# NoahVl/Explaining-In-Style-Reproducibility-Study

Measured on AMD Instinct MI355X. Metric: StylEx G+D+enc train-step images/sec @256px, higher is better.
Workload: dtype bf16; 1 GPU; FFHQ-shaped 256x256 StylEx, batch 32/GPU, GAE=2 (noise+encoder micro-steps), GP every 4th step, ResNet-18 classifier; image_size=256, batch_per_gpu=32, start_step=0, gradient_accumulate_every=2, global_batch=32, parallelism=dp1

## Files before the change

### explaining-in-style-reproducibility-study_amd/csrc/elementwise.hip

```cpp
#include <hip/hip_runtime.h>
#include <stdint.h>

#include "stylex_internal.h"

namespace {

template <int V>
struct Vec;
template <>
struct Vec<4> {
    typedef float4 T;
    static __device__ __forceinline__ T zero() { return make_float4(0.f, 0.f, 0.f, 0.f); }
    static __device__ __forceinline__ T ld(const void* p, long off, int bf) { return act_ld4(p, off, bf); }
    static __device__ __forceinline__ void st(void* p, long off, T v, int bf) { act_st4(p, off, v, bf); }
    static __device__ __forceinline__ void fma(T& a, float w, T x) {
        a.x = fmaf(w, x.x, a.x); a.y = fmaf(w, x.y, a.y); a.z = fmaf(w, x.z, a.z); a.w = fmaf(w, x.w, a.w);
    }
};
template <>
struct Vec<1> {
    typedef float T;
    static __device__ __forceinline__ T zero() { return 0.f; }
    static __device__ __forceinline__ T ld(const void* p, long off, int bf) { return act_ld1(p, off, bf); }
    static __device__ __forceinline__ void st(void* p, long off, T v, int bf) { act_st1(p, off, v, bf); }
// ... 99 lines not shown
            float ch = up_coef(oh, ih, H);
            if (ch == 0.f) continue;
#pragma unroll
            for (int e = -1; e <= 2; ++e) {
                int ow = 2 * iw + e;
                if (ow < 0 || ow >= 2 * W) continue;
                float cw = up_coef(ow, iw, W);
                if (cw == 0.f) continue;
                Vec<V>::fma(acc, ch * cw, Vec<V>::ld(dy, base + ((long)oh * 2 * W + ow) * C, bf));
            }
        }
        Vec<V>::st(dx, pix * C + c, acc, bf);
    }
}

__device__ __forceinline__ int reflect1(int i, int n) { return i < 0 ? -i : (i >= n ? 2 * n - 2 - i : i); }

__device__ __forceinline__ float ub_coef(int o, int i, int n) {
    const int n2 = 2 * n;
    return 0.25f * up_coef(reflect1(o - 1, n2), i, n) + 0.5f * up_coef(o, i, n) + 0.25f * up_coef(reflect1(o + 1, n2), i, n);
}

template <int V>
__global__ void rgb_up_blur_add_fwd_kernel(const void* __restrict__ rgb, const void* __restrict__ prev, void* __restrict__ y,
                                           int B, int H, int W, int C, int bf) {
    const int cv = C / V;
    const long total = (long)B * 2 * H * 2 * W * cv;
    for (long i = blockIdx.x * (long)blockDim.x + threadIdx.x; i < total; i += (long)gridDim.x * blockDim.x) {
        int cq, ow, oh, b;
        const long pix = decomp_index(i, cv, 2 * W, 2 * H, cq, ow, oh, b);
// ... 359 lines not shown
           ((reinterpret_cast<uintptr_t>(b) & 15) == 0);
}
template <bool ADJ>
static int launch_blur_strip(const void* in, void* out, int B, int H, int W, int C, int s2d, hipStream_t s,
                             const void* gate = nullptr, float gslope = 0.f, const void* gmask = nullptr) {
    constexpr int ROWS = 8;
    long work = (long)B * ((H + ROWS - 1) / ROWS) * W * (C / 8);
    long blocks = (work + 255) / 256;
    if (blocks > 16384) blocks = 16384;
    hipLaunchKernelGGL((blur3x3_strip_kernel<ADJ, ROWS>), dim3((unsigned)blocks), dim3(256), 0, s,
                       (const unsigned short*)in, (unsigned short*)out, B, H, W, C, s2d, (const unsigned short*)gate,
                       gslope, (const unsigned char*)gmask);
    return (int)hipGetLastError();
}

extern "C" {

#define EW_ARGS const int64_t* sh, int act_dtype, void* stream
#define EW_UNPACK                                                     \
    hipStream_t s = (hipStream_t)stream;                               \
    int B = (int)sh[0], H = (int)sh[1], W = (int)sh[2], C = (int)sh[3]; \
    int bf = act_dtype == 1;                                           \
    if (act_dtype != 0 && act_dtype != 1) return STYLEX_EINVAL;

int stylex_upsample2x_bilinear_fwd(const void* x, void* y, EW_ARGS) {
    EW_UNPACK
    if (B <= 0 || H <= 0 || W <= 0 || C <= 0) return STYLEX_EINVAL;
    LAUNCH_EW(upsample2x_fwd_kernel, (long)B * 4 * H * W * C, x, y, x, y, B, H, W, C, bf);
}
int stylex_upsample2x_bilinear_bwd(const void* dy, void* dx, EW_ARGS) {
    EW_UNPACK
    if (B <= 0 || H <= 0 || W <= 0 || C <= 0) return STYLEX_EINVAL;
    LAUNCH_EW(upsample2x_bwd_kernel, (long)B * H * W * C, dy, dx, dy, dx, B, H, W, C, bf);
}
int stylex_rgb_up_blur_add_fwd(const void* rgb, const void* prev, void* y, EW_ARGS) {
    EW_UNPACK
    if (!rgb || !y || B <= 0 || H <= 0 || W <= 0 || C <= 0) return STYLEX_EINVAL;
    const void* al = prev ? prev : rgb;
    if (vec_ok(C, rgb, y) && vec_ok(C, al, y))
        hipLaunchKernelGGL(rgb_up_blur_add_fwd_kernel<4>, dim3(grid_for((long)B * 4 * H * W * C / 4)), dim3(256), 0, s, rgb, prev,
                           y, B, H, W, C, bf);
    else
        hipLaunchKernelGGL(rgb_up_blur_add_fwd_kernel<1>, dim3(grid_for((long)B * 4 * H * W * C)), dim3(256), 0, s, rgb, prev, y,
                           B, H, W, C, bf);
    return (int)hipGetLastError();
}
int stylex_rgb_up_blur_add_bwd(const void* dy, void* dx, EW_ARGS) {
// ... 117 lines not shown
```

### explaining-in-style-reproducibility-study_amd/csrc/fused_bwd.hip

```cpp
#include <hip/hip_runtime.h>
#include <stdint.h>

#include "stylex_internal.h"

namespace {

constexpr int NT = 256;

template <int K>
struct Acc {
    float4 v[K];
    __device__ __forceinline__ void zero() {
#pragma unroll
        for (int k = 0; k < K; ++k) v[k] = make_float4(0.f, 0.f, 0.f, 0.f);
    }
};

template <int K>
__device__ __forceinline__ void block_reduce_store(Acc<K>& a, float* smem, int cv, int prow, int CV, int rpp, int C,
                                                   float* partial_row , bool active) {
    float4* s4 = reinterpret_cast<float4*>(smem);
    if (active) {
#pragma unroll
        for (int k = 0; k < K; ++k) s4[(k * rpp + prow) * CV + cv] = a.v[k];
// ... 30 lines not shown
    if (g.CV > NT) g.CV = NT;
    g.rpp = NT / g.CV;
    g.cv = threadIdx.x % g.CV;
    g.prow = threadIdx.x / g.CV;
    g.active = g.prow < g.rpp;
    g.b = blockIdx.y;
    long per = ((long)HW + nchunks - 1) / nchunks;
    g.p_begin = (long)blockIdx.x * per;
    g.p_end = g.p_begin + per < HW ? g.p_begin + per : HW;
    return g;
}

__device__ __forceinline__ float4 ld4(const void* p, long off, int bf) { return act_ld4(p, off, bf); }
__device__ __forceinline__ void st4(void* p, long off, float4 v, int bf) { act_st4(p, off, v, bf); }
__device__ __forceinline__ float4 ldp4(const float* p) { return *reinterpret_cast<const float4*>(p); }

__global__ __launch_bounds__(NT) void act_bwd_reduce_kernel(const void* __restrict__ dy, const void* __restrict__ y,
                                                           void* __restrict__ dx, float* __restrict__ partial, int HW,
                                                           int C, int nchunks, int lrelu, float scale, int bf) {
    extern __shared__ __attribute__((aligned(16))) float smem[];
    Geo g = make_geo(HW, C, nchunks);
    Acc<1> a;
    a.zero();
    const int c = g.cv * 4;
    if (g.active && c < C) {
        const long base = (long)g.b * HW;
        for (long p = g.p_begin + g.prow; p < g.p_end; p += g.rpp) {
            const long o = (base + p) * C + c;
            float4 gv = ld4(dy, o, bf);
            gv.x *= scale; gv.y *= scale; gv.z *= scale; gv.w *= scale;
// ... 6 lines not shown
                gv.w = yv.w > 0.f ? gv.w : slope * gv.w;
            }
            if (dx) st4(dx, o, gv, bf);
            a.v[0].x += gv.x; a.v[0].y += gv.y; a.v[0].z += gv.z; a.v[0].w += gv.w;
        }
    }
    block_reduce_store<1>(a, smem, g.cv, g.prow, g.CV, g.rpp, C, partial + ((long)g.b * nchunks + blockIdx.x) * C,
                          g.active && c < C);
}

__global__ __launch_bounds__(NT) void modconv_bwd_prep_kernel(const void* __restrict__ gy, const void* __restrict__ y,
                                                             const float* __restrict__ noise, int ns,
                                                             const float* __restrict__ nw, const float* __restrict__ nb,
                                                             void* __restrict__ gz, float* __restrict__ partial, int H,
                                                             int W, int C, int nchunks, int lrelu, int bf,
                                                             const float* __restrict__ gz_scale) {
    extern __shared__ __attribute__((aligned(16))) float smem[];
    const int HW = H * W;
    Geo g = make_geo(HW, C, nchunks);
    Acc<3> a;
    a.zero();
    const int c = g.cv * 4;
    if (g.active && c < C) {
        float4 w4 = make_float4(0.f, 0.f, 0.f, 0.f), b4 = w4;
        if (noise) {
            w4 = ldp4(nw + c);
            b4 = ldp4(nb + c);
        }
        float4 d4 = make_float4(1.f, 1.f, 1.f, 1.f);
        if (gz_scale) d4 = ldp4(gz_scale + (long)g.b * C + c);
        const long base = (long)g.b * HW;
        for (long p = g.p_begin + g.prow; p < g.p_end; p += g.rpp) {
            const long o = (base + p) * C + c;
            float4 gv = ld4(gy, o, bf);
            float4 yv = ld4(y, o, bf);
            float nz = 0.f;
            if (noise) {
                const int pi = (int)p, h = pi / W, w = pi - h * W;
                nz = noise[((long)g.b * ns + w) * ns + h];
            }
            float4 t = yv;
            if (lrelu) {
                gv.x = yv.x > 0.f ? gv.x : 0.2f * gv.x; t.x = yv.x > 0.f ? yv.x : 5.f * yv.x;
                gv.y = yv.y > 0.f ? gv.y : 0.2f * gv.y; t.y = yv.y > 0.f ? yv.y : 5.f * yv.y;
                gv.z = yv.z > 0.f ? gv.z : 0.2f * gv.z; t.z = yv.z > 0.f ? yv.z : 5.f * yv.z;
                gv.w = yv.w > 0.f ? gv.w : 0.2f * gv.w; t.w = yv.w > 0.f ? yv.w : 5.f * yv.w;
            }
            if (gz_scale) st4(gz, o, make_float4(gv.x * d4.x, gv.y * d4.y, gv.z * d4.z, gv.w * d4.w), bf);
            else st4(gz, o, gv, bf);
            a.v[0].x += gv.x * (t.x - (nz * w4.x + b4.x));
            a.v[0].y += gv.y * (t.y - (nz * w4.y + b4.y));
            a.v[0].z += gv.z * (t.z - (nz * w4.z + b4.z));
            a.v[0].w += gv.w * (t.w - (nz * w4.w + b4.w));
            a.v[1].x += gv.x * nz; a.v[1].y += gv.y * nz; a.v[1].z += gv.z * nz; a.v[1].w += gv.w * nz;
            a.v[2].x += gv.x; a.v[2].y += gv.y; a.v[2].z += gv.z; a.v[2].w += gv.w;
// ... 17 lines not shown
        for (long p = g.p_begin + g.prow; p < g.p_end; p += g.rpp) {
            const long o = (base + p) * C + c;
            float4 tv = ld4(t, o, bf);
            float4 xv = ld4(x, o, bf);
            a.v[0].x += xv.x * tv.x; a.v[0].y += xv.y * tv.y; a.v[0].z += xv.z * tv.z; a.v[0].w += xv.w * tv.w;
            if (gx) {
                tv.x *= s4.x; tv.y *= s4.y; tv.z *= s4.z; tv.w *= s4.w;
                st4(gx, o, tv, bf);
            }
        }
    }
    block_reduce_store<1>(a, smem, g.cv, g.prow, g.CV, g.rpp, C, partial + ((long)g.b * nchunks + blockIdx.x) * C,
                          g.active && c < C);
}

inline size_t reduce_smem(int C, int K) {
    int CV = (C + 3) / 4;
    if (CV > NT) CV = NT;
    int rpp = NT / CV;
    return (size_t)K * rpp * CV * 16;
}

inline bool ok_shape(const int64_t* sh, int nchunks) {
    return sh[0] > 0 && sh[1] > 0 && sh[2] > 0 && sh[3] > 0 && sh[3] <= 1024 && (sh[3] % 4 == 0) && nchunks > 0 &&
           sh[0] <= 65535;
}

}

extern "C" {
// ... 7 lines not shown
    return (int)n;
}

int stylex_act_bwd_reduce(const void* dy, const void* y, void* dx, float* partial, const int64_t* sh, int nchunks,
                          int lrelu, float scale, int act_dtype, void* stream) {
    if (act_dtype != 0 && act_dtype != 1) return STYLEX_EINVAL;
    if (!dy || !partial || !ok_shape(sh, nchunks) || (lrelu && !y)) return STYLEX_EINVAL;
    int HW = (int)(sh[1] * sh[2]), C = (int)sh[3];
    hipLaunchKernelGGL(act_bwd_reduce_kernel, dim3(nchunks, (unsigned)sh[0]), dim3(NT), reduce_smem(C, 1),
                       (hipStream_t)stream, dy, y, dx, partial, HW, C, nchunks, lrelu, scale, act_dtype);
    return (int)hipGetLastError();
}

static int modconv_bwd_prep_impl(const void* gy, const void* y, const float* noise, int64_t noise_stride,
                                 const float* noise_w, const float* noise_b, void* gz, float* partial, const int64_t* sh,
                                 int nchunks, int lrelu, int act_dtype, const float* gz_scale, void* stream);

int stylex_modconv_bwd_prep(const void* gy, const void* y, const float* noise, int64_t noise_stride,
                            const float* noise_w, const float* noise_b, void* gz, float* partial, const int64_t* sh,
                            int nchunks, int lrelu, int act_dtype, void* stream) {
    return modconv_bwd_prep_impl(gy, y, noise, noise_stride, noise_w, noise_b, gz, partial, sh, nchunks, lrelu, act_dtype,
                                 nullptr, stream);
}

int stylex_modconv_bwd_prep_scaled(const void* gy, const void* y, const float* noise, int64_t noise_stride,
                                   const float* noise_w, const float* noise_b, const float* gz_scale, void* gz,
                                   float* partial, const int64_t* sh, int nchunks, int lrelu, int act_dtype, void* stream) {
    if (!gz_scale || (reinterpret_cast<uintptr_t>(gz_scale) & 15)) return STYLEX_EINVAL;
    return modconv_bwd_prep_impl(gy, y, noise, noise_stride, noise_w, noise_b, gz, partial, sh, nchunks, lrelu, act_dtype,
                                 gz_scale, stream);
}

static int modconv_bwd_prep_impl(const void* gy, const void* y, const float* noise, int64_t noise_stride,
                                 const float* noise_w, const float* noise_b, void* gz, float* partial, const int64_t* sh,
                                 int nchunks, int lrelu, int act_dtype, const float* gz_scale, void* stream) {
    if (act_dtype != 0 && act_dtype != 1) return STYLEX_EINVAL;
    if (lrelu != 0 && lrelu != 1) return STYLEX_EINVAL;
    if (!gy || !y || !gz || !partial || !ok_shape(sh, nchunks)) return STYLEX_EINVAL;
    if (noise && (!noise_w || !noise_b || noise_stride < sh[1] || noise_stride < sh[2])) return STYLEX_EINVAL;
    int C = (int)sh[3];
    hipLaunchKernelGGL(modconv_bwd_prep_kernel, dim3(nchunks, (unsigned)sh[0]), dim3(NT), reduce_smem(C, 3),
                       (hipStream_t)stream, gy, y, noise, (int)noise_stride, noise_w, noise_b, gz, partial, (int)sh[1],
                       (int)sh[2], C, nchunks, lrelu, act_dtype, gz_scale);
    return (int)hipGetLastError();
}

int stylex_scale_reduce(const void* x, const void* t, const float* s, void* gx, float* partial, const int64_t* sh,
                        int nchunks, int act_dtype, void* stream) {
    if (act_dtype != 0 && act_dtype != 1) return STYLEX_EINVAL;
    if (!x || !t || !s || !partial || !ok_shape(sh, nchunks)) return STYLEX_EINVAL;
    int HW = (int)(sh[1] * sh[2]), C = (int)sh[3];
    hipLaunchKernelGGL(scale_reduce_kernel, dim3(nchunks, (unsigned)sh[0]), dim3(NT), reduce_smem(C, 1),
                       (hipStream_t)stream, x, t, s, gx, partial, HW, C, nchunks, act_dtype);
    return (int)hipGetLastError();
}

}
```

### explaining-in-style-reproducibility-study_amd/stylex/hip_backend.py

```python
import os as _os

if _os.environ.get("STYLEX_MIOPEN_ALLOW_BWD_GTC", "0") != "1":
    _os.environ.setdefault("MIOPEN_DEBUG_CONV_IMPLICIT_GEMM_ASM_BWD_GTC_XDLOPS_NHWC", "0")

import atexit
import ctypes
import os
import weakref

import torch

import operand_cache
from operand_cache import mark_updated, packs, stamp as _gen, vectors

_HERE = os.path.dirname(os.path.abspath(__file__))
LIB_PATH = os.path.join(os.path.dirname(_HERE), "libstylex_hip.so")

F32, BF16, BF16_ACT = 0, 1, 2
EPI_BIAS, EPI_LRELU, EPI_OSCALE, EPI_NOISE, EPI_RESIDUAL, EPI_RELU, EPI_GATE, EPI_NOISE_NAT = 1, 2, 4, 8, 16, 32, 64, 128
EPI_MASK_OUT, EPI_GATE_MASK = 256, 512

_c_f = ctypes.c_void_p
_i64p = ctypes.POINTER(ctypes.c_int64)

# ... 51 lines not shown
    "stylex_rgb_up_blur_add_fwd": (ctypes.c_int, [_c_f, _c_f, _c_f, _i64p, ctypes.c_int, ctypes.c_void_p]),
    "stylex_rgb_up_blur_add_bwd": (ctypes.c_int, [_c_f, _c_f, _i64p, ctypes.c_int, ctypes.c_void_p]),
    "stylex_blur3x3_reflect_fwd": (ctypes.c_int, [_c_f, _c_f, _i64p, ctypes.c_int, ctypes.c_void_p]),
    "stylex_blur3x3_reflect_bwd": (ctypes.c_int, [_c_f, _c_f, _i64p, ctypes.c_int, ctypes.c_void_p]),
    "stylex_bias_act_fwd": (ctypes.c_int, [_c_f, _c_f, _c_f, ctypes.c_int64, _c_f, _c_f, _c_f, _i64p, ctypes.c_int,
                                           ctypes.c_void_p]),
    "stylex_bias_act_bwd": (ctypes.c_int, [_c_f, _c_f, _c_f, _i64p, ctypes.c_int, ctypes.c_void_p]),
    "stylex_rowwise_sumsq": (ctypes.c_int, [_c_f, _c_f, _i64p, ctypes.c_void_p]),
    "stylex_reduce_chunks": (ctypes.c_int, [_i64p]),
    "stylex_act_bwd_reduce": (ctypes.c_int, [_c_f, _c_f, _c_f, _c_f, _i64p, ctypes.c_int, ctypes.c_int, ctypes.c_float,
                                             ctypes.c_int, ctypes.c_void_p]),
    "stylex_modconv_bwd_prep": (ctypes.c_int, [_c_f, _c_f, _c_f, ctypes.c_int64, _c_f, _c_f, _c_f, _c_f, _i64p,
                                               ctypes.c_int, ctypes.c_int, ctypes.c_int, ctypes.c_void_p]),
    "stylex_modconv_bwd_prep_scaled": (ctypes.c_int, [_c_f, _c_f, _c_f, ctypes.c_int64, _c_f, _c_f, _c_f, _c_f, _c_f, _i64p,
                                                      ctypes.c_int, ctypes.c_int, ctypes.c_int, ctypes.c_void_p]),
    "stylex_scale_reduce": (ctypes.c_int, [_c_f, _c_f, _c_f, _c_f, _c_f, _i64p, ctypes.c_int, ctypes.c_int,
                                           ctypes.c_void_p]),
    "stylex_pad_rgb8": (ctypes.c_int, [_c_f, _c_f, _i64p, _i64p, ctypes.c_int, ctypes.c_void_p]),
    "stylex_affine_act_nchw_fwd": (ctypes.c_int, [_c_f, _c_f, _c_f, _c_f, _c_f, ctypes.c_int64, ctypes.c_int64, ctypes.c_int64,
                                                  ctypes.c_int, ctypes.c_void_p]),
    "stylex_affine_act_nchw_bwd": (ctypes.c_int, [_c_f, _c_f, _c_f, _c_f, _c_f, ctypes.c_int64, ctypes.c_int64, ctypes.c_int64,
                                                  ctypes.c_int, ctypes.c_void_p]),
    "stylex_affine_relu_maxpool_fwd": (ctypes.c_int, [_c_f, _c_f, _c_f, _c_f, _c_f, ctypes.c_int64, ctypes.c_int64,
                                                      ctypes.c_int64, ctypes.c_int64, ctypes.c_void_p]),
    "stylex_affine_relu_maxpool_bwd": (ctypes.c_int, [_c_f, _c_f, _c_f, _c_f, ctypes.c_int64, ctypes.c_int64, ctypes.c_int64,
                                                      ctypes.c_int64, ctypes.c_void_p]),
    "stylex_lpips_tap_nhwc_fwd": (ctypes.c_int, [_c_f, _c_f, _c_f, _c_f, _c_f, _c_f, ctypes.c_int64, ctypes.c_int64, ctypes.c_int64,
                                                 ctypes.c_int64, ctypes.c_void_p]),
    "stylex_lpips_tap_nhwc_bwd": (ctypes.c_int, [_c_f, _c_f, _c_f, _c_f, _c_f, _c_f, _c_f, _c_f, ctypes.c_int64, ctypes.c_int64,
                                                 ctypes.c_int64, ctypes.c_void_p]),
# ... 64 lines not shown
                                               ctypes.c_void_p]),
    "stylex_crop_lut_u8": (ctypes.c_int, [ctypes.c_void_p, _c_f, ctypes.c_int64, ctypes.c_int64, ctypes.c_int64, _c_f,
                                          ctypes.c_int64, _c_f, _c_f, ctypes.c_int64, ctypes.c_void_p]),
    "stylex_timing_report": (ctypes.c_int, [ctypes.c_int, _i64p, ctypes.POINTER(ctypes.c_double),
                                            ctypes.POINTER(ctypes.c_double), ctypes.POINTER(ctypes.c_double)]),
}

_lib = None
_inited_devices = set()


class StylexHipError(RuntimeError):
    pass


def load_library(path=None):
    global _lib
    if _lib is not None:
        return _lib
    path = path or os.environ.get("STYLEX_HIP_LIB", LIB_PATH)
    if not os.path.isfile(path):
        raise StylexHipError("libstylex_hip.so not found at %s — run `python __graft_entry__.py build` "
                             "(there is no CPU fallback for the product path)" % path)
    lib = ctypes.CDLL(path)
    for name, (res, args) in SIGNATURES.items():
        fn = getattr(lib, name)
        fn.restype = res
        fn.argtypes = args
    if os.environ.get("STYLEX_SYNC_TRACE", "0") == "1":
        lib = _SyncTraced(lib)
    _lib = lib
    return lib


class _SyncTraced:

    def __init__(self, lib):
        self._lib = lib

    def __getattr__(self, name):
# ... 1173 lines not shown
    flat = not per_sample and b > 1
    if flat:
        nbytes = b * h * w * c * dy.element_size()
        h, b = b * h, 1
    shp = _shape(b, h, w, c)
    nch = lib.stylex_reduce_chunks(shp)
    if flat:
        nch = max(1, min(nch, max(64, -(-nbytes // (64 * 1024)))))
    partial = _empty((b, nch, c), dtype=torch.float32, device=dy.device)
    dx = empty_cl(tuple(dy.shape), dy) if want_dx else None
    _check(lib.stylex_act_bwd_reduce(_ptr(dy), _ptr(y), _ptr(dx), _ptr(partial), shp, nch, 2 if lrelu == "relu" else int(bool(lrelu)),
                                     float(scale), _adt(dy), _stream()), "stylex_act_bwd_reduce")
    return dx, ((partial.sum(dim=1) if per_sample else partial.sum(dim=(0, 1))) if want_sum else None)


def modconv_bwd_prep(gy, y, noise, noise_w, noise_b, lrelu, gz_scale=None):
    lib = _ensure_device(gy)
    assert is_cl(gy) and is_cl(y) and gy.dtype == y.dtype
    b, c, h, w = gy.shape
    shp = _shape(b, h, w, c)
    nch = lib.stylex_reduce_chunks(shp)
    partial = _empty((b, nch, 3, c), dtype=torch.float32, device=gy.device)
    gz = empty_cl(tuple(gy.shape), gy)
    ns = 0
    noise, noise_w, noise_b = _f32(noise), _f32(noise_w), _f32(noise_b)
    if noise is not None:
        ns = noise.shape[1]
    lr = 2 if lrelu == "relu" else int(bool(lrelu))
    if gz_scale is None:
        _check(lib.stylex_modconv_bwd_prep(_ptr(gy), _ptr(y), _ptr(noise), ns, _ptr(noise_w), _ptr(noise_b), _ptr(gz),
                                           _ptr(partial), shp, nch, lr, _adt(gy), _stream()), "stylex_modconv_bwd_prep")
    else:
        gz_scale = _f32(gz_scale)
        _check(lib.stylex_modconv_bwd_prep_scaled(_ptr(gy), _ptr(y), _ptr(noise), ns, _ptr(noise_w), _ptr(noise_b),
                                                  _ptr(gz_scale), _ptr(gz), _ptr(partial), shp, nch, lr, _adt(gy), _stream()),
               "stylex_modconv_bwd_prep_scaled")
    return gz, partial.sum(dim=1)


def scale_reduce(x, t, s, want_gx=True):
    lib = _ensure_device(x)
    assert is_cl(x) and is_cl(t) and x.dtype == t.dtype
    b, c, h, w = x.shape
    shp = _shape(b, h, w, c)
# ... 305 lines not shown
```

### explaining-in-style-reproducibility-study_amd/stylex/ops.py

```python
import collections
import math

import os

import torch
from contextlib import nullcontext as _nullcontext
import torch.nn.functional as F

import hip_backend as hb

_PRECISION = hb.F32


_NAMES = {"fp32": hb.F32, "f32": hb.F32, "bf16": hb.BF16_ACT, "bf16_f32act": hb.BF16}


def set_precision(name):
    global _PRECISION
    _PRECISION = _NAMES[name]


def get_precision():
    return {hb.F32: "fp32", hb.BF16_ACT: "bf16", hb.BF16: "bf16_f32act"}[_PRECISION]

# ... 492 lines not shown
    @staticmethod
    def forward(ctx, x, s1, d, w, noise, nw, nb, pad, lrelu, noise_nat=None):
        x = _cl(x)
        pre = _PRECISION == hb.BF16_ACT and s1 is not None and x.shape[2] * x.shape[3] <= 64 and x.shape[1] % 64 == 0
        ctx.pre = pre
        if pre:
            x_in, s_in = (x.float() * s1[:, :, None, None]).to(x.dtype).contiguous(memory_format=torch.channels_last), None
        else:
            x_in, s_in = x, s1
        if noise_nat is not None and noise_nat.shape[1] % 4 == 0:
            y = hb.conv2d_fwd(x_in, w, 1, pad, _PRECISION, in_scale=s_in, out_scale=d, noise=noise_nat, noise_w=nw,
                              noise_b=nb, lrelu=lrelu, noise_natural=True)
        else:
            y = hb.conv2d_fwd(x_in, w, 1, pad, _PRECISION, in_scale=s_in, out_scale=d, noise=noise, noise_w=nw, noise_b=nb,
                              lrelu=lrelu)
        ctx.save_for_backward(x, s1, d, w, noise, nw, nb, y if (lrelu or d is not None or noise is not None) else None)
        ctx.cfg = (pad, lrelu)
        return y

    @staticmethod
    @torch.autograd.function.once_differentiable
    def backward(ctx, gy):
        x, s1, d, w, noise, nw, nb, y = ctx.saved_tensors
        pad, lrelu = ctx.cfg
        gy = _cl(gy)
        gd = gnw = gnb = None
        folded = False
        if y is not None and _reducible(gy.shape[1]):
            fold = d is not None and _PRECISION != hb.F32 and os.environ.get("STYLEX_FOLD_D", "1") != "0"
            gz, sums = hb.modconv_bwd_prep(gy, y, noise, nw, nb, lrelu, gz_scale=d if fold else None)
            folded = fold
            if d is not None:
                gd = sums[:, 0] / d
            if noise is not None:
                gnw, gnb = sums[:, 1:3].sum(0)
        elif y is not None:
            raise hb.StylexHipError("fused modulated conv needs C_out % 4 == 0")
        else:
            gz = gy
        gx = gs1 = gw = None
        if ctx.needs_input_grad[0] or ctx.needs_input_grad[1]:
            if folded:
                t = hb.conv2d_bwd_data(gz, w, tuple(x.shape), 1, pad, _PRECISION)
            elif ctx.pre and d is not None:
                gzd = (gz.float() * d[:, :, None, None]).to(gz.dtype).contiguous(memory_format=torch.channels_last)
# ... 864 lines not shown
```

### include/stylex_hip.h

```cpp
#ifndef STYLEX_HIP_H
#define STYLEX_HIP_H

#include <stdint.h>

#ifdef __cplusplus
extern "C" {
#endif

#define STYLEX_F32 0
#define STYLEX_BF16 1
#define STYLEX_BF16_ACT 2

#define STYLEX_EINVAL (-1)
#define STYLEX_EWORKSPACE (-2)

#define STYLEX_CONV_NSHAPE 11

#define STYLEX_EPI_BIAS 1
#define STYLEX_EPI_LRELU 2
#define STYLEX_EPI_OSCALE 4
#define STYLEX_EPI_NOISE 8
#define STYLEX_EPI_RESIDUAL 16
#define STYLEX_EPI_RELU 32
#define STYLEX_EPI_NOISE_NAT 128
// ... 122 lines not shown
                        float eps, void* stream);
int stylex_modcoeff_bwd(const float* gd, const float* d, const float* s1, const float* wsq, const float* w,
                        const float* gs1, float* gstyle, float* gw, int64_t B, int64_t C, int64_t O, int64_t K,
                        void* stream);

int stylex_reduce_chunks(const int64_t* shape);
int stylex_act_bwd_reduce(const void* dy, const void* y, void* dx, float* partial, const int64_t* shape, int nchunks,
                          int lrelu, float scale, int act_dtype, void* stream);
int stylex_modconv_bwd_prep(const void* gy, const void* y, const float* noise, int64_t noise_stride,
                            const float* noise_w, const float* noise_b, void* gz, float* partial,
                            const int64_t* shape, int nchunks, int lrelu, int act_dtype, void* stream);
int stylex_modconv_bwd_prep_scaled(const void* gy, const void* y, const float* noise, int64_t noise_stride,
                                   const float* noise_w, const float* noise_b, const float* gz_scale, void* gz,
                                   float* partial, const int64_t* shape, int nchunks, int lrelu, int act_dtype,
                                   void* stream);
int stylex_scale_reduce(const void* x, const void* t, const float* s, void* gx, float* partial, const int64_t* shape,
                        int nchunks, int act_dtype, void* stream);

int stylex_torgb_chunks(const int64_t* shape);
int stylex_torgb_fwd(const void* x, const float* s1, const float* w, void* y, const int64_t* shape, void* stream);
int stylex_torgb_bwd(const void* x, const void* gy, const float* s1, const float* w, void* gx, float* partial,
                     const int64_t* shape, void* stream);

int stylex_timing_enable(int on);
int stylex_timing_pause(int on);
int stylex_timing_report(int kernel_class, int64_t* launches, double* total_ms, double* total_flops,
                         double* total_bytes);
int stylex_timing_layers(int64_t* meta, double* vals, int64_t cap);
int stylex_timing_kernels(char* names, int64_t* meta, double* vals, int64_t cap);

// ... 81 lines not shown
```

Before: 988.7 images/sec.

## Add strip-tiled bf16 upsample kernels and 8-wide modconv backward glue kernels

After: 1003 images/sec (median of 6 runs). +1.4%, better.

```diff
diff --git a/explaining-in-style-reproducibility-study_amd/csrc/elementwise.hip b/explaining-in-style-reproducibility-study_amd/csrc/elementwise.hip
--- a/explaining-in-style-reproducibility-study_amd/csrc/elementwise.hip
+++ b/explaining-in-style-reproducibility-study_amd/csrc/elementwise.hip
@@ -1,5 +1,6 @@
 #include <hip/hip_runtime.h>
 #include <stdint.h>
+#include <stdlib.h>
 
 #include "stylex_internal.h"
 
@@ -137,6 +138,115 @@
     }
 }
 
+struct UpPair {
+    F8 e, o;
+};
+template <int ROWS>
+__global__ __launch_bounds__(256) void upsample2x_fwd_strip_kernel(const unsigned short* __restrict__ x,
+                                                                   unsigned short* __restrict__ y, int B, int H, int W, int C) {
+    const int cv = C >> 3;
+    const int strips = (H + ROWS - 1) / ROWS;
+    const long total = (long)B * strips * W * cv;
+    const int rs = W * C, ors = 2 * W * C;
+    for (long i = blockIdx.x * (long)blockDim.x + threadIdx.x; i < total; i += (long)gridDim.x * blockDim.x) {
+        int cq, w, hs, b;
+        decomp_index(i, cv, W, strips, cq, w, hs, b);
+        const int h0 = hs * ROWS;
+        const unsigned short* xin = x + (long)b * H * rs + cq * 8;
+        unsigned short* yout = y + (long)b * 2 * H * ors + 2 * w * C + cq * 8;
+        const int ol = max(w - 1, 0) * C, om = w * C, orr = min(w + 1, W - 1) * C;
+        auto hpair = [&](int hh) -> UpPair {
+            const int ro = hh * rs;
+            const F8 l = Vec<8>::ld(xin, ro + ol, 1), m = Vec<8>::ld(xin, ro + om, 1), r = Vec<8>::ld(xin, ro + orr, 1);
+            UpPair p{Vec<8>::zero(), Vec<8>::zero()};
+            Vec<8>::fma(p.e, 1.f - 0.75f, l);
+            Vec<8>::fma(p.e, 0.75f, m);
+            Vec<8>::fma(p.o, 1.f - 0.25f, m);
+            Vec<8>::fma(p.o, 0.25f, r);
+            return p;
+        };
+        auto vmix = [&](float wlo, const F8& lo, float whi, const F8& hi, int off) {
+            F8 acc = Vec<8>::zero();
+            Vec<8>::fma(acc, wlo, lo);
+            Vec<8>::fma(acc, whi, hi);
+            Vec<8>::st(yout, off, acc, 1);
+        };
+        UpPair prev = hpair(max(h0 - 1, 0)), cur = hpair(h0);
+#pragma unroll
+        for (int r = 0; r < ROWS; ++r) {
+            const int h = h0 + r;
+            if (h >= H) break;
+            const UpPair next = hpair(min(h + 1, H - 1));
+            const int o0 = 2 * h * ors;
+            vmix(1.f - 0.75f, prev.e, 0.75f, cur.e, o0);
+            vmix(1.f - 0.75f, prev.o, 0.75f, cur.o, o0 + C);
+            vmix(1.f - 0.25f, cur.e, 0.25f, next.e, o0 + ors);
+            vmix(1.f - 0.25f, cur.o, 0.25f, next.o, o0 + ors + C);
+            prev = cur;
+            cur = next;
+        }
+    }
+}
+
+template <int ROWS>
+__global__ __launch_bounds__(256) void upsample2x_bwd_strip_kernel(const unsigned short* __restrict__ dy,
+                                                                   unsigned short* __restrict__ dx, int B, int H, int W, int C) {
+    const int cv = C >> 3;
+    const int strips = (H + ROWS - 1) / ROWS;
+    const long total = (long)B * strips * W * cv;
+    const int rs = W * C, ors = 2 * W * C;
+    for (long i = blockIdx.x * (long)blockDim.x + threadIdx.x; i < total; i += (long)gridDim.x * blockDim.x) {
+        int cq, iw, hs, b;
+        decomp_index(i, cv, W, strips, cq, iw, hs, b);
+        const int h0 = hs * ROWS;
+        const uint4* src = reinterpret_cast<const uint4*>(dy + (long)b * 2 * H * ors + cq * 8);
+        unsigned short* dst = dx + (long)b * H * rs + iw * C + cq * 8;
+        int oc[4];
+        float cw[4];
+#pragma unroll
+        for (int e = 0; e < 4; ++e) {
+            const int ow = 2 * iw + e - 1;
+            const bool in = ow >= 0 && ow < 2 * W;
+            cw[e] = in ? up_coef(ow, iw, W) : 0.f;
+            oc[e] = (min(max(ow, 0), 2 * W - 1) * C) >> 3;
+        }
+        auto ldrow = [&](int oh, uint4 (&v)[4]) {
+            const int ro = (min(max(oh, 0), 2 * H - 1) * ors) >> 3;
+#pragma unroll
+            for (int e = 0; e < 4; ++e) v[e] = src[ro + oc[e]];
+        };
+        uint4 win[4][4];
+        ldrow(2 * h0 - 1, win[0]);
+        ldrow(2 * h0, win[1]);
+#pragma unroll
+        for (int r = 0; r < ROWS; ++r) {
+            const int ih = h0 + r;
+            if (ih >= H) break;
+            ldrow(2 * ih + 1, win[2]);
+            ldrow(2 * ih + 2, win[3]);
+            F8 acc = Vec<8>::zero();
+#pragma unroll
+            for (int a = 0; a < 4; ++a) {
+                const int oh = 2 * ih + a - 1;
+                const float ch = (oh >= 0 && oh < 2 * H) ? up_coef(oh, ih, H) : 0.f;
+                if (ch == 0.f) continue;
+#pragma unroll
+                for (int e = 0; e < 4; ++e) {
+                    if (cw[e] == 0.f) continue;
+                    const uint4 q = win[a][e];
+                    Vec<8>::fma(acc, ch * cw[e], F8{act_unpack4(make_uint2(q.x, q.y)), act_unpack4(make_uint2(q.z, q.w))});
+                }
+            }
+            Vec<8>::st(dst, ih * rs, acc, 1);
+#pragma unroll
+            for (int e = 0; e < 4; ++e) {
+                win[0][e] = win[2][e];
+                win[1][e] = win[3][e];
+            }
+        }
+    }
+}
+
 __device__ __forceinline__ int reflect1(int i, int n) { return i < 0 ? -i : (i >= n ? 2 * n - 2 - i : i); }
 
 __device__ __forceinline__ float ub_coef(int o, int i, int n) {
@@ -526,6 +636,18 @@
     return (int)hipGetLastError();
 }
 
+constexpr int UP_ROWS = 8;
+static bool up_strip_ok(int bf, int H, int W, int C, const void* a, const void* b) {
+    const char* env = getenv("STYLEX_UPSAMPLE_STRIP");
+    return bf && (C % 8 == 0) && H >= UP_ROWS && (long)4 * H * W * C < (1L << 31) && !(env && env[0] == '0') &&
+           ((reinterpret_cast<uintptr_t>(a) & 15) == 0) && ((reinterpret_cast<uintptr_t>(b) & 15) == 0);
+}
+static unsigned up_strip_blocks(int B, int H, int W, int C) {
+    long work = (long)B * ((H + UP_ROWS - 1) / UP_ROWS) * W * (C / 8);
+    long blocks = (work + 255) / 256;
+    return (unsigned)(blocks > 16384 ? 16384 : blocks);
+}
+
 extern "C" {
 
 #define EW_ARGS const int64_t* sh, int act_dtype, void* stream
@@ -538,11 +660,21 @@
 int stylex_upsample2x_bilinear_fwd(const void* x, void* y, EW_ARGS) {
     EW_UNPACK
     if (B <= 0 || H <= 0 || W <= 0 || C <= 0) return STYLEX_EINVAL;
+    if (up_strip_ok(bf, H, W, C, x, y)) {
+        hipLaunchKernelGGL(upsample2x_fwd_strip_kernel<UP_ROWS>, dim3(up_strip_blocks(B, H, W, C)), dim3(256), 0, s,
+                           (const unsigned short*)x, (unsigned short*)y, B, H, W, C);
+        return (int)hipGetLastError();
+    }
     LAUNCH_EW(upsample2x_fwd_kernel, (long)B * 4 * H * W * C, x, y, x, y, B, H, W, C, bf);
 }
 int stylex_upsample2x_bilinear_bwd(const void* dy, void* dx, EW_ARGS) {
     EW_UNPACK
     if (B <= 0 || H <= 0 || W <= 0 || C <= 0) return STYLEX_EINVAL;
+    if (up_strip_ok(bf, H, W, C, dy, dx)) {
+        hipLaunchKernelGGL(upsample2x_bwd_strip_kernel<UP_ROWS>, dim3(up_strip_blocks(B, H, W, C)), dim3(256), 0, s,
+                           (const unsigned short*)dy, (unsigned short*)dx, B, H, W, C);
+        return (int)hipGetLastError();
+    }
     LAUNCH_EW(upsample2x_bwd_kernel, (long)B * H * W * C, dy, dx, dy, dx, B, H, W, C, bf);
 }
 int stylex_rgb_up_blur_add_fwd(const void* rgb, const void* prev, void* y, EW_ARGS) {
diff --git a/explaining-in-style-reproducibility-study_amd/csrc/fused_bwd.hip b/explaining-in-style-reproducibility-study_amd/csrc/fused_bwd.hip
--- a/explaining-in-style-reproducibility-study_amd/csrc/fused_bwd.hip
+++ b/explaining-in-style-reproducibility-study_amd/csrc/fused_bwd.hip
@@ -1,5 +1,6 @@
 #include <hip/hip_runtime.h>
 #include <stdint.h>
+#include <stdlib.h>
 
 #include "stylex_internal.h"
 
@@ -68,6 +69,27 @@
 __device__ __forceinline__ float4 ld4(const void* p, long off, int bf) { return act_ld4(p, off, bf); }
 __device__ __forceinline__ void st4(void* p, long off, float4 v, int bf) { act_st4(p, off, v, bf); }
 __device__ __forceinline__ float4 ldp4(const float* p) { return *reinterpret_cast<const float4*>(p); }
+
+struct PixWalk {
+    int h, w, dh, dw, W;
+    __device__ __forceinline__ PixWalk(int p, int step, int W_) : W(W_) {
+        h = p / W_;
+        w = p - h * W_;
+        dh = step / W_;
+        dw = step - dh * W_;
+    }
+    __device__ __forceinline__ void advance() {
+        w += dw;
+        h += dh;
+        if (w >= W) {
+            w -= W;
+            ++h;
+        }
+    }
+};
+__device__ __forceinline__ long noise_off(int b, int ns, int h, int w, int natural) {
+    return natural ? ((long)b * ns + h) * ns + w : ((long)b * ns + w) * ns + h;
+}
 
 __global__ __launch_bounds__(NT) void act_bwd_reduce_kernel(const void* __restrict__ dy, const void* __restrict__ y,
                                                            void* __restrict__ dx, float* __restrict__ partial, int HW,
@@ -104,7 +126,7 @@
                                                              const float* __restrict__ nw, const float* __restrict__ nb,
                                                              void* __restrict__ gz, float* __restrict__ partial, int H,
                                                              int W, int C, int nchunks, int lrelu, int bf,
-                                                             const float* __restrict__ gz_scale) {
+                                                             const float* __restrict__ gz_scale, int natural) {
     extern __shared__ __attribute__((aligned(16))) float smem[];
     const int HW = H * W;
     Geo g = make_geo(HW, C, nchunks);
@@ -120,15 +142,13 @@
         float4 d4 = make_float4(1.f, 1.f, 1.f, 1.f);
         if (gz_scale) d4 = ldp4(gz_scale + (long)g.b * C + c);
         const long base = (long)g.b * HW;
-        for (long p = g.p_begin + g.prow; p < g.p_end; p += g.rpp) {
+        PixWalk pw((int)(g.p_begin + g.prow), g.rpp, W);
+        for (long p = g.p_begin + g.prow; p < g.p_end; p += g.rpp, pw.advance()) {
             const long o = (base + p) * C + c;
             float4 gv = ld4(gy, o, bf);
             float4 yv = ld4(y, o, bf);
             float nz = 0.f;
-            if (noise) {
-                const int pi = (int)p, h = pi / W, w = pi - h * W;
-                nz = noise[((long)g.b * ns + w) * ns + h];
-            }
+            if (noise) nz = noise[noise_off(g.b, ns, pw.h, pw.w, natural)];
             float4 t = yv;
             if (lrelu) {
                 gv.x = yv.x > 0.f ? gv.x : 0.2f * gv.x; t.x = yv.x > 0.f ? yv.x : 5.f * yv.x;
@@ -176,6 +196,190 @@
                           g.active && c < C);
 }
 
+constexpr int NT8 = NT / 2;
+struct L8 {
+    float e[8];
+};
+__device__ __forceinline__ uint4 ldraw8(const void* p, long off) {
+    return *reinterpret_cast<const uint4*>(reinterpret_cast<const unsigned short*>(p) + off);
+}
+__device__ __forceinline__ L8 unpack8(const uint4& h) {
+    L8 r;
+    r.e[0] = act_lo(h.x); r.e[1] = act_hi(h.x); r.e[2] = act_lo(h.y); r.e[3] = act_hi(h.y);
+    r.e[4] = act_lo(h.z); r.e[5] = act_hi(h.z); r.e[6] = act_lo(h.w); r.e[7] = act_hi(h.w);
+    return r;
+}
+__device__ __forceinline__ L8 ld8(const void* p, long off) { return unpack8(ldraw8(p, off)); }
+__device__ __forceinline__ void st8(void* p, long off, const L8& v) {
+    *reinterpret_cast<uint4*>(reinterpret_cast<unsigned short*>(p) + off) =
+        make_uint4(act_pack2(v.e[0], v.e[1]), act_pack2(v.e[2], v.e[3]), act_pack2(v.e[4], v.e[5]), act_pack2(v.e[6], v.e[7]));
+}
+__device__ __forceinline__ L8 ldp8(const float* p) {
+    const float4 a = ldp4(p), b = ldp4(p + 4);
+    return L8{{a.x, a.y, a.z, a.w, b.x, b.y, b.z, b.w}};
+}
+
+struct Geo8 {
+    int b, cv, prow, CV, rpp;
+    int p_begin, p_end;
+    bool active;
+};
+__device__ __forceinline__ Geo8 make_geo8(int HW, int C, int nchunks) {
+    Geo8 g;
+    g.CV = C >> 3;
+    g.rpp = NT / (C >> 2);
+    g.cv = threadIdx.x % g.CV;
+    g.prow = threadIdx.x / g.CV;
+    g.active = g.prow < g.rpp;
+    g.b = blockIdx.y;
+    const long per = ((long)HW + nchunks - 1) / nchunks;
+    const long pb = (long)blockIdx.x * per;
+    g.p_begin = (int)(pb < HW ? pb : HW);
+    g.p_end = (int)(pb + per < HW ? pb + per : HW);
+    return g;
+}
+
+template <int K>
+__device__ __forceinline__ void block_reduce_store8(const L8 (&a)[K], float* smem, const Geo8& g, int C, float* partial_row) {
+    float4* s4 = reinterpret_cast<float4*>(smem);
+    if (g.active) {
+#pragma unroll
+        for (int k = 0; k < K; ++k) {
+            const int at = ((k * g.rpp + g.prow) * g.CV + g.cv) * 2;
+            s4[at] = make_float4(a[k].e[0], a[k].e[1], a[k].e[2], a[k].e[3]);
+            s4[at + 1] = make_float4(a[k].e[4], a[k].e[5], a[k].e[6], a[k].e[7]);
+        }
+    }
+    __syncthreads();
+    if (g.active && g.prow == 0) {
+#pragma unroll
+        for (int k = 0; k < K; ++k) {
+            float4 t = make_float4(0.f, 0.f, 0.f, 0.f), u = t;
+            for (int r = 0; r < g.rpp; ++r) {
+                const int at = ((k * g.rpp + r) * g.CV + g.cv) * 2;
+                const float4 x = s4[at], y = s4[at + 1];
+                t.x += x.x; t.y += x.y; t.z += x.z; t.w += x.w;
+                u.x += y.x; u.y += y.y; u.z += y.z; u.w += y.w;
+            }
+            float4* d = reinterpret_cast<float4*>(partial_row + (long)k * C + g.cv * 8);
+            d[0] = t;
+            d[1] = u;
+        }
+    }
+}
+
+__global__ __launch_bounds__(NT8) void modconv_bwd_prep_wide_kernel(const void* __restrict__ gy, const void* __restrict__ y,
+                                                                  const float* __restrict__ noise, int ns,
+                                                                  const float* __restrict__ nw, const float* __restrict__ nb,
+                                                                  void* __restrict__ gz, float* __restrict__ partial, int H,
+                                                                  int W, int C, int nchunks, int lrelu,
+                                                                  const float* __restrict__ gz_scale, int natural) {
+    extern __shared__ __attribute__((aligned(16))) float smem[];
+    const int HW = H * W;
+    const Geo8 g = make_geo8(HW, C, nchunks);
+    L8 a[3] = {};
+    if (g.active) {
+        const int c = g.cv * 8;
+        L8 w8 = {}, b8 = {}, d8 = {};
+        if (noise) {
+            w8 = ldp8(nw + c);
+            b8 = ldp8(nb + c);
+        }
+        if (gz_scale) d8 = ldp8(gz_scale + (long)g.b * C + c);
+        const long step = (long)g.rpp * C;
+        long o = ((long)g.b * HW + g.p_begin + g.prow) * C + c;
+        PixWalk pw(g.p_begin + g.prow, g.rpp, W);
+        for (int p = g.p_begin + g.prow; p < g.p_end; p += 2 * g.rpp, o += 2 * step, pw.advance()) {
+            const bool two = p + g.rpp < g.p_end;
+            const long o1 = two ? o + step : o;
+            const int h0 = pw.h, w0 = pw.w;
+            pw.advance();
+            const int h1 = two ? pw.h : h0, w1 = two ? pw.w : w0;
+            const L8 g0 = ld8(gy, o), g1 = ld8(gy, o1), y0 = ld8(y, o), y1 = ld8(y, o1);
+            float nz0 = 0.f, nz1 = 0.f;
+            if (noise) {
+                nz0 = noise[noise_off(g.b, ns, h0, w0, natural)];
+                nz1 = noise[noise_off(g.b, ns, h1, w1, natural)];
+            }
+            L8 q0, q1, t0 = y0, t1 = y1, s0, s1;
+#pragma unroll
+            for (int e = 0; e < 8; ++e) {
+                q0.e[e] = g0.e[e];
+                q1.e[e] = g1.e[e];
+                if (lrelu) {
+                    q0.e[e] = y0.e[e] > 0.f ? g0.e[e] : 0.2f * g0.e[e];
+                    t0.e[e] = y0.e[e] > 0.f ? y0.e[e] : 5.f * y0.e[e];
+                    q1.e[e] = y1.e[e] > 0.f ? g1.e[e] : 0.2f * g1.e[e];
+                    t1.e[e] = y1.e[e] > 0.f ? y1.e[e] : 5.f * y1.e[e];
+                }
+                s0.e[e] = gz_scale ? q0.e[e] * d8.e[e] : q0.e[e];
+                s1.e[e] = gz_scale ? q1.e[e] * d8.e[e] : q1.e[e];
+            }
+            st8(gz, o, s0);
+            if (two) st8(gz, o1, s1);
+#pragma unroll
+            for (int e = 0; e < 8; ++e) {
+                a[0].e[e] += q0.e[e] * (t0.e[e] - (nz0 * w8.e[e] + b8.e[e]));
+                a[1].e[e] += q0.e[e] * nz0;
+                a[2].e[e] += q0.e[e];
+            }
+            if (two) {
+#pragma unroll
+                for (int e = 0; e < 8; ++e) {
+                    a[0].e[e] += q1.e[e] * (t1.e[e] - (nz1 * w8.e[e] + b8.e[e]));
+                    a[1].e[e] += q1.e[e] * nz1;
+                    a[2].e[e] += q1.e[e];
+                }
+            }
+        }
+    }
+    block_reduce_store8<3>(a, smem, g, C, partial + ((long)g.b * nchunks + blockIdx.x) * 3 * C);
+}
+
+__global__ __launch_bounds__(NT8) void scale_reduce_wide_kernel(const void* __restrict__ x, const void* __restrict__ t,
+                                                              const float* __restrict__ s, void* __restrict__ gx,
+                                                              float* __restrict__ partial, int HW, int C, int nchunks) {
+    extern __shared__ __attribute__((aligned(16))) float smem[];
+    const Geo8 g = make_geo8(HW, C, nchunks);
+    L8 a[1] = {};
+    if (g.active) {
+        const int c = g.cv * 8;
+        const L8 s8 = ldp8(s + (long)g.b * C + c);
+        const long step = (long)g.rpp * C;
+        long o = ((long)g.b * HW + g.p_begin + g.prow) * C + c;
+        for (int p = g.p_begin + g.prow; p < g.p_end; p += 2 * g.rpp, o += 2 * step) {
+            const bool two = p + g.rpp < g.p_end;
+            const long o1 = two ? o + step : o;
+            L8 t0 = ld8(t, o), t1 = ld8(t, o1);
+            const L8 x0 = ld8(x, o), x1 = ld8(x, o1);
+#pragma unroll
+            for (int e = 0; e < 8; ++e) a[0].e[e] += x0.e[e] * t0.e[e];
+            if (two) {
+#pragma unroll
+                for (int e = 0; e < 8; ++e) a[0].e[e] += x1.e[e] * t1.e[e];
+            }
+            if (gx) {
+#pragma unroll
+                for (int e = 0; e < 8; ++e) {
+                    t0.e[e] *= s8.e[e];
+                    t1.e[e] *= s8.e[e];
+                }
+                st8(gx, o, t0);
+                if (two) st8(gx, o1, t1);
+            }
+        }
+    }
+    block_reduce_store8<1>(a, smem, g, C, partial + ((long)g.b * nchunks + blockIdx.x) * C);
+}
+
+inline size_t reduce_smem8(int C, int K) { return (size_t)K * (NT / (C >> 2)) * (C >> 3) * 32; }
+
+inline bool al16(const void* p) { return (reinterpret_cast<uintptr_t>(p) & 15) == 0; }
+inline bool glue_wide(int act_dtype, int C) {
+    const char* env = getenv("STYLEX_GLUE_WIDE");
+    return act_dtype == 1 && C % 8 == 0 && !(env && env[0] == '0');
+}
+
 inline size_t reduce_smem(int C, int K) {
     int CV = (C + 3) / 4;
     if (CV > NT) CV = NT;
@@ -213,13 +417,13 @@
 
 static int modconv_bwd_prep_impl(const void* gy, const void* y, const float* noise, int64_t noise_stride,
                                  const float* noise_w, const float* noise_b, void* gz, float* partial, const int64_t* sh,
-                                 int nchunks, int lrelu, int act_dtype, const float* gz_scale, void* stream);
+                                 int nchunks, int lrelu, int act_dtype, const float* gz_scale, int natural, void* stream);
 
 int stylex_modconv_bwd_prep(const void* gy, const void* y, const float* noise, int64_t noise_stride,
                             const float* noise_w, const float* noise_b, void* gz, float* partial, const int64_t* sh,
                             int nchunks, int lrelu, int act_dtype, void* stream) {
     return modconv_bwd_prep_impl(gy, y, noise, noise_stride, noise_w, noise_b, gz, partial, sh, nchunks, lrelu, act_dtype,
-                                 nullptr, stream);
+                                 nullptr, 0, stream);
 }
 
 int stylex_modconv_bwd_prep_scaled(const void* gy, const void* y, const float* noise, int64_t noise_stride,
@@ -227,20 +431,35 @@
                                    float* partial, const int64_t* sh, int nchunks, int lrelu, int act_dtype, void* stream) {
     if (!gz_scale || (reinterpret_cast<uintptr_t>(gz_scale) & 15)) return STYLEX_EINVAL;
     return modconv_bwd_prep_impl(gy, y, noise, noise_stride, noise_w, noise_b, gz, partial, sh, nchunks, lrelu, act_dtype,
-                                 gz_scale, stream);
+                                 gz_scale, 0, stream);
+}
+
+int stylex_modconv_bwd_prep_nat(const void* gy, const void* y, const float* noise, int64_t noise_stride,
+                                const float* noise_w, const float* noise_b, const float* gz_scale, void* gz, float* partial,
+                                const int64_t* sh, int nchunks, int lrelu, int act_dtype, void* stream) {
+    if (!noise || (reinterpret_cast<uintptr_t>(gz_scale) & 15)) return STYLEX_EINVAL;
+    return modconv_bwd_prep_impl(gy, y, noise, noise_stride, noise_w, noise_b, gz, partial, sh, nchunks, lrelu, act_dtype,
+                                 gz_scale, 1, stream);
 }
 
 static int modconv_bwd_prep_impl(const void* gy, const void* y, const float* noise, int64_t noise_stride,
                                  const float* noise_w, const float* noise_b, void* gz, float* partial, const int64_t* sh,
-                                 int nchunks, int lrelu, int act_dtype, const float* gz_scale, void* stream) {
+                                 int nchunks, int lrelu, int act_dtype, const float* gz_scale, int natural, void* stream) {
     if (act_dtype != 0 && act_dtype != 1) return STYLEX_EINVAL;
     if (lrelu != 0 && lrelu != 1) return STYLEX_EINVAL;
     if (!gy || !y || !gz || !partial || !ok_shape(sh, nchunks)) return STYLEX_EINVAL;
     if (noise && (!noise_w || !noise_b || noise_stride < sh[1] || noise_stride < sh[2])) return STYLEX_EINVAL;
     int C = (int)sh[3];
+    if (glue_wide(act_dtype, C) && al16(gy) && al16(y) && al16(gz) && al16(partial) && al16(noise_w) && al16(noise_b) &&
+        al16(gz_scale)) {
+        hipLaunchKernelGGL(modconv_bwd_prep_wide_kernel, dim3(nchunks, (unsigned)sh[0]), dim3(NT8), reduce_smem8(C, 3),
+                           (hipStream_t)stream, gy, y, noise, (int)noise_stride, noise_w, noise_b, gz, partial, (int)sh[1],
+                           (int)sh[2], C, nchunks, lrelu, gz_scale, natural);
+        return (int)hipGetLastError();
+    }
     hipLaunchKernelGGL(modconv_bwd_prep_kernel, dim3(nchunks, (unsigned)sh[0]), dim3(NT), reduce_smem(C, 3),
                        (hipStream_t)stream, gy, y, noise, (int)noise_stride, noise_w, noise_b, gz, partial, (int)sh[1],
-                       (int)sh[2], C, nchunks, lrelu, act_dtype, gz_scale);
+                       (int)sh[2], C, nchunks, lrelu, act_dtype, gz_scale, natural);
     return (int)hipGetLastError();
 }
 
@@ -249,6 +468,11 @@
     if (act_dtype != 0 && act_dtype != 1) return STYLEX_EINVAL;
     if (!x || !t || !s || !partial || !ok_shape(sh, nchunks)) return STYLEX_EINVAL;
     int HW = (int)(sh[1] * sh[2]), C = (int)sh[3];
+    if (glue_wide(act_dtype, C) && al16(x) && al16(t) && al16(s) && al16(gx) && al16(partial)) {
+        hipLaunchKernelGGL(scale_reduce_wide_kernel, dim3(nchunks, (unsigned)sh[0]), dim3(NT8), reduce_smem8(C, 1),
+                           (hipStream_t)stream, x, t, s, gx, partial, HW, C, nchunks);
+        return (int)hipGetLastError();
+    }
     hipLaunchKernelGGL(scale_reduce_kernel, dim3(nchunks, (unsigned)sh[0]), dim3(NT), reduce_smem(C, 1),
                        (hipStream_t)stream, x, t, s, gx, partial, HW, C, nchunks, act_dtype);
     return (int)hipGetLastError();
diff --git a/explaining-in-style-reproducibility-study_amd/stylex/hip_backend.py b/explaining-in-style-reproducibility-study_amd/stylex/hip_backend.py
--- a/explaining-in-style-reproducibility-study_amd/stylex/hip_backend.py
+++ b/explaining-in-style-reproducibility-study_amd/stylex/hip_backend.py
@@ -89,6 +89,8 @@
                                                ctypes.c_int, ctypes.c_int, ctypes.c_int, ctypes.c_void_p]),
     "stylex_modconv_bwd_prep_scaled": (ctypes.c_int, [_c_f, _c_f, _c_f, ctypes.c_int64, _c_f, _c_f, _c_f, _c_f, _c_f, _i64p,
                                                       ctypes.c_int, ctypes.c_int, ctypes.c_int, ctypes.c_void_p]),
+    "stylex_modconv_bwd_prep_nat": (ctypes.c_int, [_c_f, _c_f, _c_f, ctypes.c_int64, _c_f, _c_f, _c_f, _c_f, _c_f, _i64p,
+                                                   ctypes.c_int, ctypes.c_int, ctypes.c_int, ctypes.c_void_p]),
     "stylex_scale_reduce": (ctypes.c_int, [_c_f, _c_f, _c_f, _c_f, _c_f, _i64p, ctypes.c_int, ctypes.c_int,
                                            ctypes.c_void_p]),
     "stylex_pad_rgb8": (ctypes.c_int, [_c_f, _c_f, _i64p, _i64p, ctypes.c_int, ctypes.c_void_p]),
@@ -183,6 +185,15 @@
     pass
 
 
+OPTIONAL_SYMBOLS = frozenset(["stylex_modconv_bwd_prep_nat"])
+_MISSING_OPTIONAL = set()
+
+
+def has_symbol(name):
+    load_library()
+    return name not in _MISSING_OPTIONAL
+
+
 def load_library(path=None):
     global _lib
     if _lib is not None:
@@ -192,7 +203,11 @@
         raise StylexHipError("libstylex_hip.so not found at %s — run `python __graft_entry__.py build` "
                              "(there is no CPU fallback for the product path)" % path)
     lib = ctypes.CDLL(path)
+    _MISSING_OPTIONAL.clear()
     for name, (res, args) in SIGNATURES.items():
+        if name in OPTIONAL_SYMBOLS and path != LIB_PATH and not hasattr(lib, name):
+            _MISSING_OPTIONAL.add(name)
+            continue
         fn = getattr(lib, name)
         fn.restype = res
         fn.argtypes = args
@@ -1396,7 +1411,7 @@
     return dx, ((partial.sum(dim=1) if per_sample else partial.sum(dim=(0, 1))) if want_sum else None)
 
 
-def modconv_bwd_prep(gy, y, noise, noise_w, noise_b, lrelu, gz_scale=None):
+def modconv_bwd_prep(gy, y, noise, noise_w, noise_b, lrelu, gz_scale=None, noise_natural=False):
     lib = _ensure_device(gy)
     assert is_cl(gy) and is_cl(y) and gy.dtype == y.dtype
     b, c, h, w = gy.shape
@@ -1409,7 +1424,13 @@
     if noise is not None:
         ns = noise.shape[1]
     lr = 2 if lrelu == "relu" else int(bool(lrelu))
-    if gz_scale is None:
+    if noise_natural:
+        assert noise is not None
+        gz_scale = _f32(gz_scale)
+        _check(lib.stylex_modconv_bwd_prep_nat(_ptr(gy), _ptr(y), _ptr(noise), ns, _ptr(noise_w), _ptr(noise_b),
+                                               _ptr(gz_scale), _ptr(gz), _ptr(partial), shp, nch, lr, _adt(gy), _stream()),
+               "stylex_modconv_bwd_prep_nat")
+    elif gz_scale is None:
         _check(lib.stylex_modconv_bwd_prep(_ptr(gy), _ptr(y), _ptr(noise), ns, _ptr(noise_w), _ptr(noise_b), _ptr(gz),
                                            _ptr(partial), shp, nch, lr, _adt(gy), _stream()), "stylex_modconv_bwd_prep")
     else:
diff --git a/explaining-in-style-reproducibility-study_amd/stylex/ops.py b/explaining-in-style-reproducibility-study_amd/stylex/ops.py
--- a/explaining-in-style-reproducibility-study_amd/stylex/ops.py
+++ b/explaining-in-style-reproducibility-study_amd/stylex/ops.py
@@ -530,21 +530,26 @@
         else:
             y = hb.conv2d_fwd(x_in, w, 1, pad, _PRECISION, in_scale=s_in, out_scale=d, noise=noise, noise_w=nw, noise_b=nb,
                               lrelu=lrelu)
-        ctx.save_for_backward(x, s1, d, w, noise, nw, nb, y if (lrelu or d is not None or noise is not None) else None)
+        ctx.save_for_backward(x, s1, d, w, noise, nw, nb, y if (lrelu or d is not None or noise is not None) else None,
+                              noise_nat)
         ctx.cfg = (pad, lrelu)
         return y
 
     @staticmethod
     @torch.autograd.function.once_differentiable
     def backward(ctx, gy):
-        x, s1, d, w, noise, nw, nb, y = ctx.saved_tensors
+        x, s1, d, w, noise, nw, nb, y, noise_nat = ctx.saved_tensors
         pad, lrelu = ctx.cfg
         gy = _cl(gy)
         gd = gnw = gnb = None
         folded = False
         if y is not None and _reducible(gy.shape[1]):
             fold = d is not None and _PRECISION != hb.F32 and os.environ.get("STYLEX_FOLD_D", "1") != "0"
-            gz, sums = hb.modconv_bwd_prep(gy, y, noise, nw, nb, lrelu, gz_scale=d if fold else None)
+            if noise_nat is not None and hb.has_symbol("stylex_modconv_bwd_prep_nat"):
+                gz, sums = hb.modconv_bwd_prep(gy, y, noise_nat, nw, nb, lrelu, gz_scale=d if fold else None,
+                                               noise_natural=True)
+            else:
+                gz, sums = hb.modconv_bwd_prep(gy, y, noise, nw, nb, lrelu, gz_scale=d if fold else None)
             folded = fold
             if d is not None:
                 gd = sums[:, 0] / d
diff --git a/include/stylex_hip.h b/include/stylex_hip.h
--- a/include/stylex_hip.h
+++ b/include/stylex_hip.h
@@ -160,6 +160,10 @@
                                    const float* noise_w, const float* noise_b, const float* gz_scale, void* gz,
                                    float* partial, const int64_t* shape, int nchunks, int lrelu, int act_dtype,
                                    void* stream);
+int stylex_modconv_bwd_prep_nat(const void* gy, const void* y, const float* noise, int64_t noise_stride,
+                                const float* noise_w, const float* noise_b, const float* gz_scale, void* gz,
+                                float* partial, const int64_t* shape, int nchunks, int lrelu, int act_dtype,
+                                void* stream);
 int stylex_scale_reduce(const void* x, const void* t, const float* s, void* gx, float* partial, const int64_t* shape,
                         int nchunks, int act_dtype, void* stream);
 
```
